# impromptuRong/hd_yolo

Hardware: NVIDIA B200
Metric: postproc_tiles_per_s (higher is better)
Workload: dtype f32

## Files before the change

### hd_yolo_b200/csrc/merge.cu

```cuda
#include "hdy_common.cuh"

namespace hdy {

enum : uint8_t { MS_UNKNOWN = 0, MS_KEPT = 1, MS_SUPPRESSED = 2, MS_DROPPED = 3, MS_REMOTE_UNKNOWN = 4 };

constexpr int kMergeThreads = 256;
constexpr int kMaxRounds = 64;
constexpr float kMergeCellMargin = 1.01f;
constexpr float kMergeMaxScaled = 1.0e6f;

constexpr int kExtBins = 128;
struct MergeStats {
  float ext_sum;
  unsigned ext_cnt;
  float cell_size;
  unsigned ext_hist[kExtBins];
  int unknown[kMaxRounds + 1];
  int rounds_run;
};

constexpr int kScanThreads = 1024;
constexpr int kScanItems = 4;
constexpr int kScanTile = kScanThreads * kScanItems;

// ... 546 lines not shown
    kept_dom = __any_sync(0xffffffffu, kept_dom);
    unk_dom = __any_sync(0xffffffffu, unk_dom);
    if (lane == 0) {
      if (kept_dom)
        vstate[p] = (uint8_t)MS_SUPPRESSED;
      else if (!unk_dom)
        vstate[p] = (uint8_t)MS_KEPT;
      else
        atomicAdd(&stats->unknown[round], 1);
    }
  }
}

__global__ void __launch_bounds__(kMergeThreads) merge_large_push_kernel(const float4* __restrict__ cbox,
                                                                         const uint64_t* __restrict__ ckey,
                                                                         uint8_t* cstate, const int* __restrict__ cell,
                                                                         const MergeStats* stats, int G, float thr,
                                                                         int round, uint32_t* __restrict__ blocked) {
  if (round > 0 && stats->unknown[round - 1] == 0) return;
  const int NB = G * G + 1;
  const int n_active = cell[NB - 1];
  const int large_begin = cell[NB - 2];
  const CellGeom g = cell_geom(stats);
  volatile uint8_t* vstate = cstate;
  const int lane = threadIdx.x & 31;
  const int warp = (blockIdx.x * blockDim.x + threadIdx.x) >> 5, n_warps = (gridDim.x * blockDim.x) >> 5;
  const uint32_t stamp = (uint32_t)round + 1u;
  for (int q = large_begin + warp; q < n_active; q += n_warps) {
    const uint8_t sq = vstate[q];
    if (sq != MS_KEPT && sq != MS_UNKNOWN && sq != MS_REMOTE_UNKNOWN) continue;
    const float4 bq = cbox[q];
    const uint64_t kq = ckey[q];
    auto visit = [&](int p) {
      if (kq < ckey[p] && vstate[p] == MS_UNKNOWN && iou_gt(bq, cbox[p], thr)) {
        if (sq == MS_KEPT)
          vstate[p] = (uint8_t)MS_SUPPRESSED;
        else
          blocked[p] = stamp;
      }
    };
    const float half = 0.5f * g.cell_size;
    const float fx0 = floorf((bq.x - half) * g.inv_cell), fx1 = floorf((bq.z + half) * g.inv_cell);
    const float fy0 = floorf((bq.y - half) * g.inv_cell), fy1 = floorf((bq.w + half) * g.inv_cell);
    const bool finite = fabsf(fx0) < 1.0e9f && fabsf(fx1) < 1.0e9f && fabsf(fy0) < 1.0e9f && fabsf(fy1) < 1.0e9f &&
                        fx1 >= fx0 && fy1 >= fy0;
    if (!finite) {
      for (int p = lane; p < large_begin; p += 32) visit(p);
    } else {
      const int ix0 = (int)fx0, iy0 = (int)fy0;
      const int nx = (int)fminf(fx1 - fx0 + 1.0f, (float)G), ny = (int)fminf(fy1 - fy0 + 1.0f, (float)G);
      const long long cells = (long long)nx * ny;
      for (long long c = lane; c < cells; c += 32) {
        const int cy = (int)(c / nx), cx = (int)(c - (long long)cy * nx);
        const int b = ((ix0 + cx) & (G - 1)) + ((iy0 + cy) & (G - 1)) * G;
        const int beg = b ? cell[b - 1] : 0, end = cell[b];
        for (int p = beg; p < end; ++p) visit(p);
      }
    }
  }
}

__global__ void merge_finish_kernel(const uint32_t* __restrict__ pos, const uint8_t* __restrict__ cstate,
                                    const long long* __restrict__ n_dev, long long n_max,
                                    uint8_t* __restrict__ state, int32_t* __restrict__ status) {
  const long long n = n_dev ? min(*n_dev, n_max) : n_max;
  bool bad = false;
  for (long long i = (long long)blockIdx.x * blockDim.x + threadIdx.x; i < n; i += (long long)gridDim.x * blockDim.x) {
    const uint32_t p = pos[i];
    if (p == 0xffffffffu) continue;
    uint8_t s = cstate[p];
    if (s == MS_UNKNOWN || s == MS_REMOTE_UNKNOWN) {
      s = MS_UNKNOWN;
      bad = true;
    }
    state[i] = s;
  }
  if (bad && status) atomicOr(status, HDY_STATUS_ROUNDS);
}

constexpr int kSelThreads = 256;
constexpr int kSelMaxBlocks = 4096;

__global__ void __launch_bounds__(kSelThreads) select_count_kernel(const uint8_t* __restrict__ state,
                                                                   const long long* __restrict__ n_dev,
                                                                   long long n_max, long long chunk,
                                                                   int* __restrict__ block_counts) {
  const long long n = n_dev ? min(*n_dev, n_max) : n_max;
  const long long lo = (long long)blockIdx.x * chunk, hi = min(lo + chunk, n);
  int c = 0;
  for (long long i = lo + threadIdx.x; i < hi; i += kSelThreads) c += state[i] == MS_KEPT;
  __shared__ int part[kSelThreads / 32];
#pragma unroll
  for (int o = 16; o > 0; o >>= 1) c += __shfl_xor_sync(0xffffffffu, c, o);
  if ((threadIdx.x & 31) == 0) part[threadIdx.x >> 5] = c;
  __syncthreads();
  if (threadIdx.x == 0) {
    int t = 0;
    for (int w = 0; w < kSelThreads / 32; ++w) t += part[w];
    block_counts[blockIdx.x] = t;
  }
}

__global__ void __launch_bounds__(1024) select_scan_kernel(int* __restrict__ block_counts, int nblocks,
                                                           int* __restrict__ count_out) {
  __shared__ int warp_tmp[33];
  int v[4], s = 0;
#pragma unroll
  for (int j = 0; j < 4; ++j) {
    const int i = threadIdx.x * 4 + j;
    v[j] = i < nblocks ? block_counts[i] : 0;
    s += v[j];
  }
  int total;
  int excl = block_scan_1024(s, warp_tmp, total);
#pragma unroll
  for (int j = 0; j < 4; ++j) {
    const int i = threadIdx.x * 4 + j;
    if (i < nblocks) block_counts[i] = excl;
    excl += v[j];
  }
  if (threadIdx.x == 0) *count_out = total;
}

__global__ void __launch_bounds__(kSelThreads) select_write_kernel(const uint8_t* __restrict__ state,
                                                                   const float* __restrict__ scores,
                                                                   const long long* __restrict__ n_dev,
                                                                   long long n_max, long long chunk,
                                                                   const int* __restrict__ block_offsets,
                                                                   uint64_t* __restrict__ keys) {
  __shared__ int wcount[kSelThreads / 32];
  const long long n = n_dev ? min(*n_dev, n_max) : n_max;
  const long long lo = (long long)blockIdx.x * chunk, hi = min(lo + chunk, n);
  const int lane = threadIdx.x & 31, warp = threadIdx.x >> 5;
  long long running = block_offsets[blockIdx.x];
  for (long long i0 = lo; i0 < hi; i0 += kSelThreads) {
    const long long i = i0 + threadIdx.x;
    const bool k = i < hi && state[i] == MS_KEPT;
    const unsigned m = __ballot_sync(0xffffffffu, k);
    if (lane == 0) wcount[warp] = __popc(m);
    __syncthreads();
    int before = 0, total = 0;
#pragma unroll
    for (int w = 0; w < kSelThreads / 32; ++w) {
      const int c = wcount[w];
      if (w < warp) before += c;
      total += c;
    }
    if (k) keys[running + before + __popc(m & ((1u << lane) - 1u))] = make_key(scores[i], (uint32_t)i);
    running += total;
    __syncthreads();
  }
}

constexpr int kSortThreads = 256;
constexpr int kSortPerWarp = 1024;
constexpr int kSortWarps = kSortThreads / 32;

__global__ void __launch_bounds__(kSortThreads) sort_hist_kernel(const uint64_t* __restrict__ keys,
                                                                  const int* __restrict__ n_dev, int n_max, int shift,
                                                                  int n_sub, int* __restrict__ hist) {
  __shared__ int h[kSortWarps][256];
  const int n = n_dev ? min(*n_dev, n_max) : n_max;
  const int warp = threadIdx.x >> 5, lane = threadIdx.x & 31;
  const int sub = blockIdx.x * kSortWarps + warp;
  for (int d = lane; d < 256; d += 32) h[warp][d] = 0;
  __syncwarp();
  const long long b = (long long)sub * kSortPerWarp;
  for (int k = lane; k < kSortPerWarp; k += 32)
    if (b + k < n) atomicAdd(&h[warp][(int)((keys[b + k] >> shift) & 255)], 1);
  __syncwarp();
  if (sub < n_sub)
    for (int d = lane; d < 256; d += 32) hist[(size_t)d * n_sub + sub] = h[warp][d];
}

__global__ void __launch_bounds__(kSortThreads) sort_scatter_kernel(const uint64_t* __restrict__ keys,
                                                                     const int* __restrict__ n_dev, int n_max,
                                                                     int shift, int n_sub, const int* __restrict__ hist,
                                                                     uint64_t* __restrict__ out) {
  __shared__ int base[kSortWarps][256];
  const int n = n_dev ? min(*n_dev, n_max) : n_max;
  const int warp = threadIdx.x >> 5, lane = threadIdx.x & 31;
  const int sub = blockIdx.x * kSortWarps + warp;
  if (sub >= n_sub) return;
  for (int d = lane; d < 256; d += 32) base[warp][d] = hist[(size_t)d * n_sub + sub];
  __syncwarp();
  const long long b = (long long)sub * kSortPerWarp;
  for (int k0 = 0; k0 < kSortPerWarp; k0 += 32) {
    const long long i = b + k0 + lane;
    const bool valid = i < n;
    const uint64_t key = valid ? keys[i] : 0;
    const int d = valid ? (int)((key >> shift) & 255) : 256 + lane;
    const unsigned peers = __match_any_sync(0xffffffffu, d);
    const int rank = __popc(peers & ((1u << lane) - 1u));
    int dst = 0;
    if (valid) dst = base[warp][d] + rank;
    __syncwarp();
    if (valid && rank == 0) base[warp][d] += __popc(peers);
    __syncwarp();
    if (valid) out[dst] = key;
  }
}

__global__ void merge_gather_kernel(const uint64_t* __restrict__ keys, const int* __restrict__ count, int max_det,
                                    const float4* __restrict__ boxes, const float* __restrict__ scores,
                                    const int64_t* __restrict__ labels, int64_t* __restrict__ out_idx,
                                    float4* __restrict__ out_boxes, float* __restrict__ out_scores,
                                    int64_t* __restrict__ out_labels, int* __restrict__ out_count) {
  const int k = min(*count, max_det);
  if (blockIdx.x == 0 && threadIdx.x == 0) *out_count = k;
  for (int j = blockIdx.x * blockDim.x + threadIdx.x; j < k; j += gridDim.x * blockDim.x) {
    const uint32_t i = key_index(keys[j]);
    if (out_idx) out_idx[j] = (int64_t)i;
    if (out_boxes) out_boxes[j] = boxes[i];
    if (out_scores) out_scores[j] = scores[i];
    if (out_labels && labels) out_labels[j] = labels[i];
  }
}

static inline unsigned blocks_for(long long n, int threads, int max_blocks = 148 * 16) {
  long long b = (n + threads - 1) / threads;
  if (b < 1) b = 1;
  if (b > max_blocks) b = max_blocks;
  return (unsigned)b;
}

constexpr int kSeamHdr = HDY_SEAM_HDR_WORDS, kSeamFar = HDY_SEAM_FAR_WORDS, kSeamRow = HDY_SEAM_ROW_WORDS;
constexpr int kSeamMaxWorld = HDY_SEAM_MAX_WORLD;
enum { SM_NTOTAL = 0, SM_MARGIN = 2, SM_GBASE = 3, SM_FLAGS = 4, SM_FAR_TOTAL = 5, SM_UNDECIDED = 8, SM_REP_OFF = 16,
       SM_OWN_SEAM = 88 };

__device__ __forceinline__ void atomic_min_float(float* addr, float v) {
  if (v >= 0.f)
    atomicMin(reinterpret_cast<int*>(addr), __float_as_int(v));
  else
    atomicMax(reinterpret_cast<unsigned*>(addr), __float_as_uint(v));
}
__device__ __forceinline__ void atomic_max_float(float* addr, float v) {
  if (v >= 0.f)
    atomicMax(reinterpret_cast<int*>(addr), __float_as_int(v));
  else
    atomicMin(reinterpret_cast<unsigned*>(addr), __float_as_uint(v));
}

__global__ void seam_summary_pack_kernel(long long n_local, const float* __restrict__ margin,
                                         const float4* __restrict__ far_boxes, const int32_t* __restrict__ far_tile,
                                         const int32_t* __restrict__ far_count, int far_list_capacity, int tile_base,
                                         int far_cap, int32_t* __restrict__ block) {
  const int k = blockIdx.x * blockDim.x + threadIdx.x;
  const int nf = far_count ? *far_count : 0;
  if (k == 0) {
    float* f = reinterpret_cast<float*>(block);
    const float big = 3.0e38f;
    f[0] = big, f[1] = big, f[2] = -big, f[3] = -big;
    f[4] = margin ? *margin : 0.f;
    block[5] = nf > far_list_capacity ? far_cap + 1 : nf;
    *reinterpret_cast<long long*>(block + 6) = n_local;
    for (int i = 8; i < kSeamHdr; ++i) block[i] = 0;
  }
  if (k < far_cap) {
    int32_t* e = block + kSeamHdr + k * kSeamFar;
    if (k < min(nf, far_list_capacity)) {
      const float4 b = far_boxes[k];
      e[0] = __float_as_int(b.x), e[1] = __float_as_int(b.y), e[2] = __float_as_int(b.z), e[3] = __float_as_int(b.w);
      e[4] = far_tile[k] + tile_base;
    } else {
      e[0] = e[1] = e[2] = e[3] = 0, e[4] = -1;
    }
    e[5] = e[6] = e[7] = 0;
  }
}

__global__ void seam_rect_kernel(const float4* __restrict__ boxes, long long n, float* __restrict__ rect) {
  const float big = 3.0e38f;
  float x1 = big, y1 = big, x2 = -big, y2 = -big;
  for (long long i = (long long)blockIdx.x * blockDim.x + threadIdx.x; i < n; i += (long long)gridDim.x * blockDim.x) {
    const float4 b = boxes[i];
    x1 = fminf(x1, fmaxf(b.x, -big)), y1 = fminf(y1, fmaxf(b.y, -big));
    x2 = fmaxf(x2, fminf(b.z, big)), y2 = fmaxf(y2, fminf(b.w, big));
  }
#pragma unroll
  for (int o = 16; o > 0; o >>= 1) {
    x1 = fminf(x1, __shfl_xor_sync(0xffffffffu, x1, o)), y1 = fminf(y1, __shfl_xor_sync(0xffffffffu, y1, o));
    x2 = fmaxf(x2, __shfl_xor_sync(0xffffffffu, x2, o)), y2 = fmaxf(y2, __shfl_xor_sync(0xffffffffu, y2, o));
  }
  if ((threadIdx.x & 31) == 0 && x2 >= x1) {
    atomic_min_float(rect + 0, x1), atomic_min_float(rect + 1, y1);
    atomic_max_float(rect + 2, x2), atomic_max_float(rect + 3, y2);
  }
}

struct SeamRects {
  float4 r[kSeamMaxWorld];
  int live[kSeamMaxWorld];
};
__device__ __forceinline__ void seam_load_rects(SeamRects& S, const int32_t* summaries, int world, int rank, int hb) {
  for (int q = threadIdx.x; q < world; q += blockDim.x) {
    const int32_t* h = summaries + (size_t)q * hb;
    S.r[q] = make_float4(__int_as_float(h[0]), __int_as_float(h[1]), __int_as_float(h[2]), __int_as_float(h[3]));
    S.live[q] = (q != rank) && (*reinterpret_cast<const long long*>(h + 6) > 0);
  }
  __syncthreads();
}
__device__ __forceinline__ bool seam_row(const float4& b, const SeamRects& S, int world) {
  bool s = false;
  for (int q = 0; q < world; ++q)
    s |= S.live[q] && (b.z >= S.r[q].x) && (b.x <= S.r[q].z) && (b.w >= S.r[q].y) && (b.y <= S.r[q].w);
  return s;
}

__global__ void __launch_bounds__(kSelThreads) seam_count_kernel(const float4* __restrict__ boxes, long long n,
                                                                 long long chunk, const int32_t* __restrict__ summaries,
                                                                 int world, int rank, int hb,
                                                                 int* __restrict__ block_counts) {
  __shared__ SeamRects S;
  __shared__ int part[kSelThreads / 32];
  seam_load_rects(S, summaries, world, rank, hb);
  const long long lo = (long long)blockIdx.x * chunk, hi = min(lo + chunk, n);
  int c = 0;
  for (long long i = lo + threadIdx.x; i < hi; i += kSelThreads) c += seam_row(boxes[i], S, world);
#pragma unroll
  for (int o = 16; o > 0; o >>= 1) c += __shfl_xor_sync(0xffffffffu, c, o);
  if ((threadIdx.x & 31) == 0) part[threadIdx.x >> 5] = c;
  __syncthreads();
  if (threadIdx.x == 0) {
    int t = 0;
    for (int w = 0; w < kSelThreads / 32; ++w) t += part[w];
    block_counts[blockIdx.x] = t;
  }
}

__global__ void __launch_bounds__(kSelThreads) seam_write_kernel(const float4* __restrict__ boxes,
                                                                 const float* __restrict__ scores, long long n,
                                                                 long long chunk, const int32_t* __restrict__ summaries,
                                                                 int world, int rank, int hb,
                                                                 const int* __restrict__ block_offsets, int seam_cap,
                                                                 int32_t* __restrict__ sel, int32_t* __restrict__ block) {
  __shared__ SeamRects S;
  __shared__ int wcount[kSelThreads / 32];
  seam_load_rects(S, summaries, world, rank, hb);
  long long gbase = 0;
  for (int q = 0; q < rank; ++q) gbase += *reinterpret_cast<const long long*>(summaries + (size_t)q * hb + 6);
  const long long lo = (long long)blockIdx.x * chunk, hi = min(lo + chunk, n);
  const int lane = threadIdx.x & 31, warp = threadIdx.x >> 5;
  long long running = block_offsets[blockIdx.x];
  for (long long i0 = lo; i0 < hi; i0 += kSelThreads) {
    const long long i = i0 + threadIdx.x;
    float4 b = make_float4(0.f, 0.f, 0.f, 0.f);
    bool k = false;
    if (i < hi) {
      b = boxes[i];
      k = seam_row(b, S, world);
    }
    const unsigned m = __ballot_sync(0xffffffffu, k);
    if (lane == 0) wcount[warp] = __popc(m);
    __syncthreads();
    int before = 0, total = 0;
#pragma unroll
    for (int w = 0; w < kSelThreads / 32; ++w) {
      const int c = wcount[w];
      if (w < warp) before += c;
      total += c;
    }
    const long long slot = running + before + __popc(m & ((1u << lane) - 1u));
    if (k && slot < seam_cap) {
      sel[slot] = (int32_t)i;
      int32_t* e = block + kSeamHdr + slot * kSeamRow;
      e[0] = __float_as_int(b.x), e[1] = __float_as_int(b.y), e[2] = __float_as_int(b.z), e[3] = __float_as_int(b.w);
      e[4] = __float_as_int(scores[i]);
// ... 268 lines not shown
      set_error("hdy_seam_select: %s", cudaGetErrorString(e));
      return HDY_ERR_CUDA;
    }
    return HDY_OK;
  }
  HDY_REQUIRE(boxes && scores && ((uintptr_t)boxes & 15) == 0, "hdy_seam_select: NULL or misaligned pointer");
  long long chunk = (n_local + kSelMaxBlocks - 1) / kSelMaxBlocks;
  chunk = ((chunk + kSelThreads - 1) / kSelThreads) * kSelThreads;
  if (chunk < 4 * kSelThreads) chunk = 4 * kSelThreads;
  const int nblocks = (int)((n_local + chunk - 1) / chunk);
  const float4* b4 = reinterpret_cast<const float4*>(boxes);
  const int hb = seam_hb(far_cap);
  seam_count_kernel<<<nblocks, kSelThreads, 0, st>>>(b4, n_local, chunk, summaries, world, rank, hb, block_scratch);
  select_scan_kernel<<<1, 1024, 0, st>>>(block_scratch, nblocks, block_scratch + kSelMaxBlocks);
  seam_block_header_kernel<<<1, 32, 0, st>>>(block_scratch + kSelMaxBlocks, block);
  seam_write_kernel<<<nblocks, kSelThreads, 0, st>>>(b4, scores, n_local, chunk, summaries, world, rank, hb,
                                                     block_scratch, seam_cap, sel, block);
  return check_launch("hdy_seam_select");
}

int hdy_seam_scatter(const int32_t* payloads, const int32_t* summaries, int world, int rank, int far_cap, int seam_cap,
                     int64_t n_local, int64_t rep_cap, float* boxes, float* scores, uint32_t* rep_gidx, int32_t* meta,
                     hdy_stream_t stream) {
  HDY_REQUIRE(world >= 1 && world <= kSeamMaxWorld && rank >= 0 && rank < world && far_cap >= 0 && seam_cap >= 0 &&
                  n_local >= 0 && rep_cap >= 0,
              "hdy_seam_scatter: bad arguments");
  HDY_REQUIRE(payloads && summaries && boxes && scores && rep_gidx && meta && ((uintptr_t)boxes & 15) == 0,
              "hdy_seam_scatter: NULL or misaligned pointer");
  dim3 grid((unsigned)(seam_cap / 1024 + 1), (unsigned)world);
  if (grid.x > 64) grid.x = 64;
  seam_scatter_kernel<<<grid, 256, 0, (cudaStream_t)stream>>>(payloads, summaries, world, rank, seam_hb(far_cap),
                                                            seam_pb(seam_cap), far_cap, seam_cap, n_local, rep_cap,
                                                            reinterpret_cast<float4*>(boxes), scores, rep_gidx, meta);
  return check_launch("hdy_seam_scatter");
}

int hdy_seam_dirty_tiles(const int32_t* summaries, int world, int far_cap, const float* tile_rois, int n_tiles,
                         uint8_t* dirty, hdy_stream_t stream) {
  HDY_REQUIRE(world >= 1 && far_cap >= 0 && n_tiles >= 0, "hdy_seam_dirty_tiles: bad sizes");
  if (n_tiles == 0) return HDY_OK;
  HDY_REQUIRE(summaries && tile_rois && dirty && ((uintptr_t)tile_rois & 15) == 0,
              "hdy_seam_dirty_tiles: NULL or misaligned pointer");
  seam_dirty_tiles_kernel<<<(unsigned)((n_tiles + 127) / 128), 128, 0, (cudaStream_t)stream>>>(
      summaries, world, seam_hb(far_cap), far_cap, reinterpret_cast<const float4*>(tile_rois), n_tiles, dirty);
  return check_launch("hdy_seam_dirty_tiles");
}

int hdy_seam_build(const float* boxes, const float* scores, const uint32_t* rep_gidx, const int32_t* meta,
                   const int32_t* tile_id, int tile_base, const float* tile_cores, const uint8_t* tile_dirty,
                   int64_t n_max, int64_t n_local, float conf_thres, float iou_thres, uint8_t* state, void* workspace,
                   size_t workspace_bytes, hdy_stream_t stream) {
  HDY_REQUIRE(meta && rep_gidx, "hdy_seam_build: NULL pointer");
  MergeIn in;
  in.boxes = reinterpret_cast<const float4*>(boxes);
  in.scores = scores;
  in.rep_gidx = rep_gidx;
  in.gidx_base_dev = reinterpret_cast<const uint32_t*>(meta + SM_GBASE);
  in.tile_base = tile_base;
  in.tile_id = tile_id;
  in.tile_cores = reinterpret_cast<const float4*>(tile_cores);
  in.tile_dirty = tile_dirty;
  in.margin = reinterpret_cast<const float*>(meta + SM_MARGIN);
  in.n_dev = reinterpret_cast<const long long*>(meta + SM_NTOTAL);
  in.n_max = n_max;
  in.n_local = n_local;
  in.conf = conf_thres;
  in.thr = iou_thres;
  return merge_build_common("hdy_seam_build", in, tile_cores, state, workspace, workspace_bytes, (cudaStream_t)stream);
}

int hdy_seam_export(void* workspace, int64_t n_max, const uint8_t* state, const int32_t* sel, const int32_t* my_block,
                    int seam_cap, uint8_t* out, hdy_stream_t stream) {
  HDY_REQUIRE(workspace && n_max >= 0 && seam_cap >= 0, "hdy_seam_export: bad arguments");
  if (seam_cap == 0 || n_max == 0) return HDY_OK;
  HDY_REQUIRE(state && sel && my_block && out, "hdy_seam_export: NULL pointer");
  MergeWs w = merge_layout(workspace, n_max);
  seam_export_kernel<<<blocks_for(seam_cap, 256, 148), 256, 0, (cudaStream_t)stream>>>(w.pos, w.cstate, state, sel,
                                                                                    my_block, seam_cap, out);
  return check_launch("hdy_seam_export");
}

int hdy_seam_import(void* workspace, int64_t n_max, int64_t n_local, const uint8_t* states, const int32_t* payloads,
                    int32_t* meta, int world, int rank, int seam_cap, int exchange, hdy_stream_t stream) {
  HDY_REQUIRE(workspace && n_max >= 0 && n_local >= 0 && world >= 1 && world <= kSeamMaxWorld && rank >= 0 &&
                  rank < world && seam_cap >= 0 && exchange >= 0,
              "hdy_seam_import: bad arguments");
  HDY_REQUIRE(states && payloads && meta, "hdy_seam_import: NULL pointer");
  MergeWs w = merge_layout(workspace, n_max > 0 ? n_max : 1);
  dim3 grid((unsigned)(seam_cap / 1024 + 1), (unsigned)world);
  if (grid.x > 64) grid.x = 64;
  seam_import_kernel<<<grid, 256, 0, (cudaStream_t)stream>>>(w.pos, w.cstate, n_local, states, payloads,
                                                           seam_pb(seam_cap), meta, world, rank, seam_cap, exchange);
  return check_launch("hdy_seam_import");
}

int hdy_merge_rounds(void* workspace, int64_t n_max, float iou_thres, int first_round, int n_rounds,
                     hdy_stream_t stream) {
  HDY_REQUIRE(workspace && n_max >= 0, "hdy_merge_rounds: bad arguments");
  HDY_REQUIRE(first_round >= 0 && n_rounds >= 0 && first_round + n_rounds <= kMaxRounds,
              "hdy_merge_rounds: at most %d rounds in total", kMaxRounds);
  if (n_max == 0) return HDY_OK;
  MergeWs w = merge_layout(workspace, n_max);
  const unsigned blocks = blocks_for(n_max, kMergeThreads, 148 * 8);
  for (int r = first_round; r < first_round + n_rounds; ++r) {
    merge_large_push_kernel<<<148 * 2, kMergeThreads, 0, (cudaStream_t)stream>>>(w.cbox, w.ckey, w.cstate, w.cell,
                                                                                 w.stats, w.G, iou_thres, r, w.blocked);
    merge_round_kernel<<<blocks, kMergeThreads, 0, (cudaStream_t)stream>>>(w.cbox, w.ckey, w.cstate, w.cell, w.stats,
                                                                           w.G, iou_thres, r, w.blocked, w.ctile);
    merge_round_large_kernel<<<148 * 2, kMergeThreads, 0, (cudaStream_t)stream>>>(w.cbox, w.ckey, w.cstate, w.cell,
                                                                                  w.stats, w.G, iou_thres, r);
  }
  return check_launch("hdy_merge_rounds");
}

int hdy_merge_finish(void* workspace, const int64_t* n_dev, int64_t n_max, uint8_t* state, int32_t* status,
                     hdy_stream_t stream) {
  HDY_REQUIRE(workspace && n_max >= 0, "hdy_merge_finish: bad arguments");
  if (n_max == 0) return HDY_OK;
  HDY_REQUIRE(state != nullptr, "hdy_merge_finish: state is NULL");
  MergeWs w = merge_layout(workspace, n_max);
  merge_finish_kernel<<<blocks_for(n_max, 256), 256, 0, (cudaStream_t)stream>>>(
      w.pos, w.cstate, reinterpret_cast<const long long*>(n_dev), n_max, state, status);
  return check_launch("hdy_merge_finish");
}

int hdy_merge_nms(const float* boxes, const float* scores, const int32_t* tile_id, const float* tile_cores,
                  const uint8_t* tile_dirty, const float* margin, const int64_t* n_dev, int64_t n_max, float conf_thres,
                  float iou_thres,
                  int max_rounds, uint8_t* state, int32_t* status, void* workspace, size_t workspace_bytes,
                  hdy_stream_t stream) {
  HDY_REQUIRE(max_rounds >= 1 && max_rounds <= kMaxRounds, "hdy_merge_nms: max_rounds out of range [1,%d]", kMaxRounds);
  MergeIn in;
  in.boxes = reinterpret_cast<const float4*>(boxes);
  in.scores = scores;
  in.rep_gidx = nullptr;
  in.gidx_base_dev = nullptr;
  in.tile_base = 0;
  in.tile_id = tile_id;
  in.tile_cores = reinterpret_cast<const float4*>(tile_cores);
  in.tile_dirty = tile_dirty;
  in.margin = margin;
  in.n_dev = reinterpret_cast<const long long*>(n_dev);
  in.n_max = n_max;
  in.n_local = n_max;
  in.conf = conf_thres;
  in.thr = iou_thres;
  int rc = merge_build_common("hdy_merge_nms", in, tile_cores, state, workspace, workspace_bytes, (cudaStream_t)stream);
  if (rc) return rc;
  rc = hdy_merge_rounds(workspace, n_max, iou_thres, 0, max_rounds, stream);
  if (rc) return rc;
  return hdy_merge_finish(workspace, n_dev, n_max, state, status, stream);
}

size_t hdy_sort_workspace_bytes(int64_t n_max) {
  if (n_max <= 0) return 256;
  const long long n_sub = (n_max + kSortPerWarp - 1) / kSortPerWarp;
  const long long hist = 256 * n_sub;
  return align256((size_t)hist * 4) + align256(scan_scratch_ints(hist) * 4);
}

int hdy_sort_keys_bytes(uint64_t* keys, uint64_t* tmp, const int32_t* n_dev, int64_t n_max, int first_byte,
                        int n_bytes, void* workspace, size_t workspace_bytes, hdy_stream_t stream) {
  HDY_REQUIRE(first_byte >= 0 && n_bytes >= 0 && first_byte + n_bytes <= 8 && (n_bytes & 1) == 0,
              "hdy_sort_keys_bytes: bytes [%d, %d) -- an even number of bytes inside the key", first_byte,
              first_byte + n_bytes);
  HDY_REQUIRE(n_max >= 0 && n_max < (1ll << 31), "hdy_sort_keys_bytes: bad size");
  if (n_max == 0) return HDY_OK;
  HDY_REQUIRE(keys && tmp && workspace && workspace_bytes >= hdy_sort_workspace_bytes(n_max),
              "hdy_sort_keys_bytes: NULL pointer or workspace too small");
  cudaStream_t st = (cudaStream_t)stream;
  const int n_sub = (int)((n_max + kSortPerWarp - 1) / kSortPerWarp);
  const long long hist_n = 256ll * n_sub;
  int* hist = static_cast<int*>(workspace);
  int* scratch = reinterpret_cast<int*>(static_cast<unsigned char*>(workspace) + align256((size_t)hist_n * 4));
  const unsigned blocks = (unsigned)((n_sub + kSortWarps - 1) / kSortWarps);
  uint64_t* src = keys;
  uint64_t* dst = tmp;
  for (int pass = first_byte; pass < first_byte + n_bytes; ++pass) {
    sort_hist_kernel<<<blocks, kSortThreads, 0, st>>>(src, n_dev, (int)n_max, pass * 8, n_sub, hist);
    int rc = device_exclusive_scan(hist, hist_n, scratch, nullptr, st);
    if (rc) return rc;
    sort_scatter_kernel<<<blocks, kSortThreads, 0, st>>>(src, n_dev, (int)n_max, pass * 8, n_sub, hist, dst);
    uint64_t* t = src;
    src = dst;
    dst = t;
  }
  return check_launch("hdy_sort_keys_bytes");
}

int hdy_merge_select_ordered(const uint8_t* state, const float* scores, const int64_t* n_dev, int64_t n_max,
                             uint64_t* keys, int32_t* count, int32_t* block_scratch, hdy_stream_t stream) {
  HDY_REQUIRE(n_max >= 0 && n_max < (1ll << 31) && count && block_scratch, "hdy_merge_select_ordered: bad arguments");
  cudaStream_t st = (cudaStream_t)stream;
  if (n_max == 0) {
    cudaError_t e = cudaMemsetAsync(count, 0, 4, st);
    if (e != cudaSuccess) {
      set_error("hdy_merge_select_ordered: %s", cudaGetErrorString(e));
      return HDY_ERR_CUDA;
    }
    return HDY_OK;
  }
  HDY_REQUIRE(state && scores && keys, "hdy_merge_select_ordered: NULL pointer");
  long long chunk = (n_max + kSelMaxBlocks - 1) / kSelMaxBlocks;
  chunk = ((chunk + kSelThreads - 1) / kSelThreads) * kSelThreads;
  if (chunk < 4 * kSelThreads) chunk = 4 * kSelThreads;
  const int nblocks = (int)((n_max + chunk - 1) / chunk);
  const long long* nd = reinterpret_cast<const long long*>(n_dev);
  select_count_kernel<<<nblocks, kSelThreads, 0, st>>>(state, nd, n_max, chunk, block_scratch);
  select_scan_kernel<<<1, 1024, 0, st>>>(block_scratch, nblocks, count);
  select_write_kernel<<<nblocks, kSelThreads, 0, st>>>(state, scores, nd, n_max, chunk, block_scratch, keys);
  return check_launch("hdy_merge_select_ordered");
}

int hdy_merge_gather(const uint64_t* keys, const int32_t* count, int64_t max_det, const float* boxes,
                     const float* scores, const int64_t* labels, int64_t* out_idx, float* out_boxes,
                     float* out_scores, int64_t* out_labels, int32_t* out_count, hdy_stream_t stream) {
  HDY_REQUIRE(max_det >= 0 && max_det < (1ll << 31) && keys && count && out_count, "hdy_merge_gather: bad arguments");
  HDY_REQUIRE((!out_boxes || boxes) && (!out_scores || scores), "hdy_merge_gather: output without its source");
  HDY_REQUIRE((((uintptr_t)boxes | (uintptr_t)out_boxes) & 15) == 0, "hdy_merge_gather: box arrays must be 16-byte aligned");
  merge_gather_kernel<<<blocks_for(max_det > 0 ? max_det : 1, 256), 256, 0, (cudaStream_t)stream>>>(
      keys, count, (int)max_det, reinterpret_cast<const float4*>(boxes), scores, labels, out_idx,
      reinterpret_cast<float4*>(out_boxes), out_scores, out_labels, out_count);
  return check_launch("hdy_merge_gather");
}

}
```

### hd_yolo_b200/slide.py

```python
from __future__ import annotations

import ctypes as C
from typing import Dict, List, Optional, Sequence, Tuple

import torch

from . import _lib
from ._lib import HdyError, ptr
from .ops import DetectBatch, _Scratch, _aligned16, _call, _conf_thr_f32, _iou_thr_f32, _need_cuda, _stream

__all__ = ["sliding_window_scanner", "tile_cores", "merge_outputs", "rescale_outputs", "scale_coords", "clip_coords",
           "merge_nms", "ensemble_merge", "Ensemble", "SlideAccumulator", "sort_keys", "kept_digest", "fold_digest",
           "mask_digest",
           "STATE_KEPT", "STATE_SUPPRESSED", "STATE_DROPPED"]

STATE_UNKNOWN, STATE_KEPT, STATE_SUPPRESSED, STATE_DROPPED = 0, 1, 2, 3
AFFINE_UNPAD, AFFINE_SCALE, AFFINE_CLIP, AFFINE_ROUND = 1, 2, 4, 8
_ws = _Scratch()


def _pair(v):
    return (v, v) if isinstance(v, (int, float)) else (v[0], v[1])


def sliding_window_scanner(image_size, roi_size=None, overlap=0) -> torch.Tensor:
    if roi_size is None:
        return torch.tensor([[0., 0., image_size[0], image_size[1]]], dtype=torch.float32)
    h, w = _pair(image_size)
    roi_h, roi_w = _pair(roi_size)
    xs = torch.arange(0, w, roi_w - overlap, dtype=torch.float32) if w > roi_w else torch.zeros(1)
    ys = torch.arange(0, h, roi_h - overlap, dtype=torch.float32) if h > roi_h else torch.zeros(1)
    x0 = xs.repeat(len(ys))
    y0 = ys.repeat_interleave(len(xs))
    out = torch.stack((x0, y0, x0 + roi_w, y0 + roi_h), 1)
    out[:, 0::2] = out[:, 0::2].clamp(min=0, max=w)
    out[:, 1::2] = out[:, 1::2].clamp(min=0, max=h)
    return out


def tile_cores(rois: torch.Tensor) -> torch.Tensor:
    r = rois.detach().cpu().to(torch.float64)
    big = 3.0e38
    out = torch.empty((len(r), 4), dtype=torch.float64)
    for lo, hi in ((0, 2), (1, 3)):
        starts = torch.unique(r[:, lo])
        ends = torch.stack([r[r[:, lo] == s, hi].max() for s in starts])
        idx = torch.searchsorted(starts, r[:, lo].contiguous())
        prev_end = torch.cat([torch.tensor([-big], dtype=torch.float64), ends[:-1]])
        prev_end = torch.cummax(prev_end, 0).values
        next_start = torch.cat([starts[1:], torch.tensor([big], dtype=torch.float64)])
        out[:, lo] = prev_end[idx]
        out[:, hi] = next_start[idx]
    return out.to(torch.float32)


def _affine(rows: torch.Tensor, pad_x, pad_y, gain, scale, clip_w, clip_h, flags):
    _need_cuda(rows, "coords")
    if rows.dim() != 2 or rows.shape[1] < 4 or rows.stride(1) != 1:
        raise HdyError("coords must be [n, >=4] with unit stride along columns")
    if rows.shape[0]:
        _call("hdy_affine_boxes", ptr(rows), rows.shape[0], rows.stride(0), float(pad_x), float(pad_y), float(gain),
              float(scale), float(clip_w), float(clip_h), flags, _stream())
    return rows


def clip_coords(boxes: torch.Tensor, shape) -> None:
    _affine(boxes, 0, 0, 1, 1, shape[1], shape[0], AFFINE_CLIP)


def scale_coords(img1_shape, coords: torch.Tensor, img0_shape, ratio_pad=None, round_: bool = False) -> torch.Tensor:
    img1_shape, img0_shape = _pair(img1_shape), _pair(img0_shape)
    if ratio_pad is None:
        gain = min(img1_shape[0] / img0_shape[0], img1_shape[1] / img0_shape[1])
        pad = (img1_shape[1] - img0_shape[1] * gain) / 2, (img1_shape[0] - img0_shape[0] * gain) / 2
    else:
        gain = ratio_pad[0][0]
        pad = ratio_pad[1]
    return _affine(coords, pad[0], pad[1], gain, 1, img0_shape[1], img0_shape[0],
                   AFFINE_UNPAD | AFFINE_CLIP | (AFFINE_ROUND if round_ else 0))


def rescale_outputs(r: Dict[str, torch.Tensor], scale: float = 1.0) -> Dict[str, torch.Tensor]:
    if scale != 1.0:
        _affine(r['boxes'], 0, 0, 1, scale, 0, 0, AFFINE_SCALE)
    return r


def merge_nms(boxes: torch.Tensor, scores: torch.Tensor, conf_thres: float, iou_thres: float,
              tile_id: Optional[torch.Tensor] = None, cores: Optional[torch.Tensor] = None,
              margin: Optional[torch.Tensor] = None, n_dev: Optional[torch.Tensor] = None,
              max_rounds: int = 8, dirty: Optional[torch.Tensor] = None) -> torch.Tensor:
    _need_cuda(boxes, "boxes")
    _need_cuda(scores, "scores")
    n = boxes.shape[0]
    if boxes.dim() != 2 or boxes.shape[1] != 4 or scores.shape != (n,):
        raise HdyError("boxes must be [n,4] and scores [n]")
    dev = boxes.device
    state = torch.empty((n,), dtype=torch.uint8, device=dev)
    if n == 0:
        return state
    boxes = _aligned16(boxes.contiguous())
    scores = scores.contiguous()
    lib = _lib.load()
    wbytes = lib.hdy_merge_workspace_bytes(n)
    ws = _ws.get(dev, "merge", wbytes)
    status = torch.zeros((1,), dtype=torch.int32, device=dev)
    use_cores = cores is not None
    if use_cores and (tile_id is None or margin is None):
        raise HdyError("the interior shortcut needs tile_id, cores and margin")
    rounds = max_rounds
    while True:
        _call("hdy_merge_nms", ptr(boxes), ptr(scores), ptr(tile_id) if use_cores else None,
              ptr(cores) if use_cores else None, ptr(dirty) if use_cores else None,
              ptr(margin) if use_cores else None, ptr(n_dev), n,
              _conf_thr_f32(conf_thres), _iou_thr_f32(iou_thres), rounds, ptr(state), ptr(status), ptr(ws), wbytes,
              _stream(), launches=8 + 3 * rounds)
        if not int(status.item()) & _lib.HDY_STATUS_ROUNDS:
            return state
        if rounds >= 64:
            raise HdyError("merge NMS did not converge in 64 rounds")
        rounds, _ = min(64, rounds * 2), status.zero_()


def dirty_tiles(far_boxes: torch.Tensor, far_tile: torch.Tensor, far_count: torch.Tensor,
                rois: torch.Tensor) -> torch.Tensor:
    n_tiles = int(rois.shape[0])
    dirty = torch.empty((max(n_tiles, 1),), dtype=torch.uint8, device=rois.device)
    _call("hdy_merge_dirty_tiles", ptr(far_boxes), ptr(far_tile), ptr(far_count), int(far_boxes.shape[0]),
          ptr(_aligned16(rois.contiguous())), n_tiles, ptr(dirty), _stream())
    return dirty


def sort_keys(keys: torch.Tensor, n_dev: Optional[torch.Tensor] = None, first_byte: int = 0,
              n_bytes: int = 8) -> torch.Tensor:
    if not keys.is_cuda or keys.dtype != torch.int64 or not keys.is_contiguous():
        raise HdyError("keys must be a contiguous CUDA int64 tensor")
    n = keys.numel()
    if n:
        lib = _lib.load()
        wbytes = lib.hdy_sort_workspace_bytes(n)
        ws = _ws.get(keys.device, "sort", wbytes)
        tmp = _ws.get(keys.device, "sort_tmp", n * 8)
        _call("hdy_sort_keys_bytes", ptr(keys), ptr(tmp), ptr(n_dev), n, int(first_byte), int(n_bytes), ptr(ws), wbytes,
              _stream(), launches=int(n_bytes) * 5)
    return keys


def _order_keys(state, scores, n: int, count: torch.Tensor) -> torch.Tensor:
    dev = scores.device
    keys = torch.empty((max(n, 1),), dtype=torch.int64, device=dev)
    if n == 0:
        count.zero_()
        return keys
    blk = _ws.get(dev, "select_blocks", 4096 * 4)
    _call("hdy_merge_select_ordered", ptr(state), ptr(scores), None, n, ptr(keys), ptr(count), ptr(blk), _stream(),
          launches=3)
    sort_keys(keys, n_dev=count, first_byte=4, n_bytes=4)
    return keys


def _gather_ordered(keys, count, k_all: int, max_det: int, boxes, scores, labels):
    dev = boxes.device
    k = min(int(k_all), int(max_det))
    idx = torch.empty((k,), dtype=torch.int64, device=dev)
    ob = torch.empty((k, 4), dtype=torch.float32, device=dev)
    os_ = torch.empty((k,), dtype=torch.float32, device=dev)
    ol = torch.empty((k,), dtype=torch.int64, device=dev) if labels is not None else None
    oc = torch.empty((1,), dtype=torch.int32, device=dev)
    if k:
        _call("hdy_merge_gather", ptr(keys), ptr(count), k, ptr(boxes), ptr(scores), ptr(labels), ptr(idx), ptr(ob),
              ptr(os_), ptr(ol), ptr(oc), _stream())
    return idx, ob, os_, ol


def _kept_in_order(state, boxes, scores, labels, max_det: int, n_dev=None):
    n = boxes.shape[0]
    count = torch.empty((1,), dtype=torch.int32, device=boxes.device)
    keys = _order_keys(state, scores, n, count)
    return _gather_ordered(keys, count, int(count.item()), max_det, boxes, scores, labels)


def kept_digest(state: torch.Tensor, base: int = 0) -> torch.Tensor:
    idx = torch.nonzero(state == STATE_KEPT).flatten().to(torch.int64) + int(base)
    h = idx * -7046029254386353131
    h = h ^ (h >> 31)
    h = h * -4658895280553007687
    h = h ^ (h >> 29)
    lo = (h & 0xffffffff).sum()
    hi = ((h >> 32) & 0xffffffff).sum()
    return torch.stack([torch.tensor(idx.numel(), dtype=torch.int64, device=state.device), lo, hi])


def fold_digest(t: torch.Tensor) -> Dict[str, object]:
    c, lo, hi = [int(v) for v in t.tolist()]
    return {"kept": c, "hash": f"{(lo + (hi << 32)) & 0xffffffffffffffff:016x}"}


def mask_digest(masks, state: torch.Tensor, base: int = 0, chunk_rows: int = 1 << 19) -> torch.Tensor:
    dev = state.device
    all_rows = torch.nonzero(state == STATE_KEPT).flatten()
    acc = torch.zeros((3,), dtype=torch.int64, device=dev)
    for c0 in range(0, int(all_rows.numel()), chunk_rows):
        rows = all_rows[c0:c0 + chunk_rows]
        g = masks.geom[rows].to(torch.int64)
        words = ((g[:, 2] + 31) >> 5) * g[:, 3]
        total = int(words.sum())
        if total == 0:
            continue
        owner = torch.repeat_interleave(torch.arange(rows.numel(), device=dev), words)
        start = torch.cumsum(words, 0) - words
        j = torch.arange(total, device=dev) - start[owner]
        w = masks.bits[masks.offsets[rows][owner] + j].to(torch.int64) & 0xffffffff
        h = ((rows[owner] + int(base)) * 1000003 + j) * -7046029254386353131
        h = (h ^ (h >> 31)) + w * -4658895280553007687
        h = h ^ (h >> 29)
        pop = w - ((w >> 1) & 0x55555555)
        pop = (pop & 0x33333333) + ((pop >> 2) & 0x33333333)
        pop = ((((pop + (pop >> 4)) & 0x0f0f0f0f) * 0x01010101) >> 24) & 0xff
        acc += torch.stack([pop.sum(), (h & 0xffffffff).sum(), ((h >> 32) & 0xffffffff).sum()])
    return acc


def merge_outputs(r: List[Dict[str, torch.Tensor]]) -> Dict[str, torch.Tensor]:
    if not len(r):
        raise HdyError("merge_outputs needs at least one tile")
    dev = r[0]['boxes'].device
    _need_cuda(r[0]['boxes'], "boxes")
    counts_h = [int(t['boxes'].shape[0]) for t in r]
    bs, md = len(r), max(max(counts_h), 1)
    n = sum(counts_h)
    res = {'labels': torch.cat([t['labels'] for t in r]), 'scores': torch.cat([t['scores'] for t in r])}
    cat = _aligned16(torch.cat([t['boxes'] for t in r]).contiguous())
    rois = torch.stack([torch.as_tensor(t['roi'], dtype=torch.float32).reshape(-1)[:4].cpu() for t in r]).to(dev)
    out = torch.empty((n, 4), dtype=torch.float32, device=dev)
    if n:
        counts = torch.tensor(counts_h, dtype=torch.int32).to(dev)
        offs = torch.tensor([0] + counts_h[:-1], dtype=torch.int64).cumsum(0).to(dev)
        tile_of = torch.repeat_interleave(torch.arange(bs, device=dev), counts.long())
        slot = torch.arange(n, device=dev) - offs[tile_of]
        padded = torch.zeros((bs, md, 4), dtype=torch.float32, device=dev)
        padded[tile_of, slot] = cat
        cursor = torch.zeros((1,), dtype=torch.int64, device=dev)
        tile_offsets = torch.empty((bs + 1,), dtype=torch.int64, device=dev)
        status = torch.zeros((1,), dtype=torch.int32, device=dev)
        for b0 in range(0, bs, 65535):
            b1 = min(bs, b0 + 65535)
            _call("hdy_merge_append", ptr(padded[b0:b1]), None, None, None, ptr(counts[b0:b1]), ptr(rois[b0:b1]), b1 - b0, md,
                  b0, 1.0, n, ptr(out), None, None, None, ptr(cursor), ptr(tile_offsets[b0:]), ptr(status), _stream(),
                  launches=2)
    res = {'boxes': out, **res}
    if 'masks' in r[0]:
        res['masks'] = torch.cat([t['masks'] for t in r])
    return res


def ensemble_merge(x: List[Dict[str, Dict[str, torch.Tensor]]], nms_params: Dict[str, float]):
    task_ids = set().union(*x)
    res: Dict[str, Dict[str, torch.Tensor]] = {}
    conf, iou, max_det = nms_params['conf_thres'], nms_params['iou_thres'], int(nms_params['max_det'])
    for task_id in task_ids:
        parts = [r[task_id] for r in x if task_id in r]
        boxes = torch.cat([p['boxes'] for p in parts])
        scores = torch.cat([p['scores'] for p in parts])
        labels = torch.cat([p['labels'] for p in parts])
        masks = None
        if any('masks' in p for p in parts):
            ref = [p['masks'] for p in parts if 'masks' in p][0]
            masks = torch.cat([p['masks'] if 'masks' in p else torch.zeros(ref.shape[1:]).to(ref.device, ref.dtype)
                               for p in parts])
        if scores.dim() != 1:
            raise HdyError("Ensemble.merge handles single-label outputs (scores [n]); the reference's multi-label "
                           "merge is unfinished (yolo.py:145)")
        lab64 = labels.to(torch.int64).contiguous()
        boxes = _aligned16(boxes.contiguous().float())
        state = merge_nms(boxes, scores.contiguous(), conf, iou)
        idx, ob, os_, ol = _kept_in_order(state, boxes, scores.contiguous(), lab64, max_det)
        out = {'boxes': ob, 'scores': os_, 'labels': ol.to(labels.dtype)}
        if masks is not None:
            out['masks'] = masks[idx]
        res[task_id] = out
    return res


class Ensemble:

    def __init__(self, models=(), nms_params: Dict[str, float] = {}):
        self.models = list(models)
        self.nms_params = self.get_nms_params(nms_params)

    def get_nms_params(self, args={}):
        default_args = {'conf_thres': 0.15, 'iou_thres': 0.45, 'max_det': 300}
        return {k: float(args.get(k, v)) for k, v in default_args.items()}

    def merge(self, x):
        return ensemble_merge(x, self.nms_params)


# ... 148 lines not shown
```

Before: 161,400.

## Replace per-pass radix sort with onesweep decoupled-lookback sort and batch gather

Replaces the per-byte histogram, device scan and scatter passes with a single upfront multi-byte histogram, a small bases kernel, and one onesweep kernel per byte. That kernel uses decoupled lookback over per-tile status words and stages keys in shared memory so global writes are coalesced. This removes the repeated scans and kernel launches for each digit pass. The gather kernel now processes several rows per thread and reads the score from the sort key instead of the scores array. The lookback spin relies on forward progress between tiles, acquired in ticket order, and the gather assumes key scores are nonzero and finite.

```diff
diff --git a/hd_yolo_b200/csrc/merge.cu b/hd_yolo_b200/csrc/merge.cu
--- a/hd_yolo_b200/csrc/merge.cu
+++ b/hd_yolo_b200/csrc/merge.cu
@@ -722,68 +722,230 @@
   }
 }
 
+constexpr int kHistThreads = 256;
+constexpr int kHistItems = 4;
+constexpr int kHistCopies = 4;
 constexpr int kSortThreads = 256;
-constexpr int kSortPerWarp = 1024;
 constexpr int kSortWarps = kSortThreads / 32;
-
-__global__ void __launch_bounds__(kSortThreads) sort_hist_kernel(const uint64_t* __restrict__ keys,
-                                                                  const int* __restrict__ n_dev, int n_max, int shift,
-                                                                  int n_sub, int* __restrict__ hist) {
-  __shared__ int h[kSortWarps][256];
+constexpr int kSortItems = 12;
+constexpr int kSortWarpKeys = kSortItems * 32;
+constexpr int kSortTile = kSortThreads * kSortItems;
+constexpr int kSortMaxBytes = 8;
+constexpr size_t kSortHdrBytes = (kSortMaxBytes * 256 + kSortMaxBytes) * 4;
+
+__device__ __forceinline__ void status_store(unsigned long long* p, unsigned long long v) {
+  asm volatile("st.relaxed.gpu.global.u64 [%0], %1;" ::"l"(p), "l"(v) : "memory");
+}
+__device__ __forceinline__ unsigned long long status_load(const unsigned long long* p) {
+  unsigned long long v;
+  asm volatile("ld.relaxed.gpu.global.u64 %0, [%1];" : "=l"(v) : "l"(p) : "memory");
+  return v;
+}
+
+__global__ void __launch_bounds__(kHistThreads) sort_hist_kernel(const uint64_t* __restrict__ keys,
+                                                                  const int* __restrict__ n_dev, int n_max,
+                                                                  int first_byte, int n_bytes,
+                                                                  unsigned* __restrict__ counts) {
+  extern __shared__ unsigned hcnt[];
   const int n = n_dev ? min(*n_dev, n_max) : n_max;
-  const int warp = threadIdx.x >> 5, lane = threadIdx.x & 31;
-  const int sub = blockIdx.x * kSortWarps + warp;
-  for (int d = lane; d < 256; d += 32) h[warp][d] = 0;
-  __syncwarp();
-  const long long b = (long long)sub * kSortPerWarp;
-  for (int k = lane; k < kSortPerWarp; k += 32)
-    if (b + k < n) atomicAdd(&h[warp][(int)((keys[b + k] >> shift) & 255)], 1);
-  __syncwarp();
-  if (sub < n_sub)
-    for (int d = lane; d < 256; d += 32) hist[(size_t)d * n_sub + sub] = h[warp][d];
-}
-
-__global__ void __launch_bounds__(kSortThreads) sort_scatter_kernel(const uint64_t* __restrict__ keys,
-                                                                     const int* __restrict__ n_dev, int n_max,
-                                                                     int shift, int n_sub, const int* __restrict__ hist,
-                                                                     uint64_t* __restrict__ out) {
-  __shared__ int base[kSortWarps][256];
+  for (int i = threadIdx.x; i < n_bytes * 256 * kHistCopies; i += kHistThreads) hcnt[i] = 0u;
+  __syncthreads();
+  const int copy = threadIdx.x % kHistCopies;
+  const long long step = (long long)gridDim.x * kHistThreads * kHistItems;
+  for (long long i0 = (long long)blockIdx.x * kHistThreads * kHistItems + threadIdx.x; i0 < n; i0 += step) {
+    uint64_t k[kHistItems];
+#pragma unroll
+    for (int e = 0; e < kHistItems; ++e) {
+      const long long i = i0 + (long long)e * kHistThreads;
+      k[e] = i < n ? keys[i] >> (8 * first_byte) : 0ull;
+    }
+#pragma unroll
+    for (int e = 0; e < kHistItems; ++e) {
+      if (i0 + (long long)e * kHistThreads >= n) break;
+      for (int b = 0; b < n_bytes; ++b)
+        atomicAdd(&hcnt[(b * 256 + (int)((k[e] >> (8 * b)) & 255ull)) * kHistCopies + copy], 1u);
+    }
+  }
+  __syncthreads();
+  for (int i = threadIdx.x; i < n_bytes * 256; i += kHistThreads) {
+    unsigned s = 0u;
+#pragma unroll
+    for (int c = 0; c < kHistCopies; ++c) s += hcnt[i * kHistCopies + c];
+    if (s) atomicAdd(&counts[i], s);
+  }
+}
+
+__global__ void __launch_bounds__(kSortMaxBytes * 32) sort_bases_kernel(unsigned* __restrict__ counts, int n_bytes) {
+  const int w = threadIdx.x >> 5, lane = threadIdx.x & 31;
+  if (w >= n_bytes) return;
+  unsigned* c = counts + w * 256 + lane * 8;
+  unsigned v[8], sum = 0u;
+#pragma unroll
+  for (int j = 0; j < 8; ++j) {
+    v[j] = c[j];
+    sum += v[j];
+  }
+  unsigned incl = sum;
+#pragma unroll
+  for (int o = 1; o < 32; o <<= 1) {
+    const unsigned u = __shfl_up_sync(0xffffffffu, incl, o);
+    if (lane >= o) incl += u;
+  }
+  unsigned run = incl - sum;
+#pragma unroll
+  for (int j = 0; j < 8; ++j) {
+    c[j] = run;
+    run += v[j];
+  }
+}
+
+__global__ void __launch_bounds__(kSortThreads, 3) sort_onesweep_kernel(const uint64_t* __restrict__ src,
+                                                                         uint64_t* __restrict__ dst,
+                                                                         const int* __restrict__ n_dev, int n_max,
+                                                                         int shift, unsigned stamp,
+                                                                         const unsigned* __restrict__ bases,
+                                                                         unsigned* __restrict__ ticket,
+                                                                         unsigned long long* __restrict__ status) {
+  __shared__ uint64_t stage[kSortTile];
+  __shared__ uint16_t whist[kSortWarps][256];
+  __shared__ int dstart[256];
+  __shared__ int gshift[256];
+  __shared__ int wsum[kSortWarps];
+  __shared__ int s_tile;
+  const int t = threadIdx.x, lane = t & 31, w = t >> 5;
+  if (t == 0) s_tile = (int)atomicAdd(ticket, 1u);
+  {
+    uint32_t* z = reinterpret_cast<uint32_t*>(&whist[0][0]);
+    for (int i = t; i < kSortWarps * 128; i += kSortThreads) z[i] = 0u;
+  }
+  __syncthreads();
+  const int tile = s_tile;
   const int n = n_dev ? min(*n_dev, n_max) : n_max;
-  const int warp = threadIdx.x >> 5, lane = threadIdx.x & 31;
-  const int sub = blockIdx.x * kSortWarps + warp;
-  if (sub >= n_sub) return;
-  for (int d = lane; d < 256; d += 32) base[warp][d] = hist[(size_t)d * n_sub + sub];
-  __syncwarp();
-  const long long b = (long long)sub * kSortPerWarp;
-  for (int k0 = 0; k0 < kSortPerWarp; k0 += 32) {
-    const long long i = b + k0 + lane;
-    const bool valid = i < n;
-    const uint64_t key = valid ? keys[i] : 0;
-    const int d = valid ? (int)((key >> shift) & 255) : 256 + lane;
-    const unsigned peers = __match_any_sync(0xffffffffu, d);
-    const int rank = __popc(peers & ((1u << lane) - 1u));
-    int dst = 0;
-    if (valid) dst = base[warp][d] + rank;
+  const long long lo = (long long)tile * kSortTile;
+  if (lo >= n) return;
+  const int in_tile = (int)min((long long)kSortTile, (long long)n - lo);
+
+  uint64_t k[kSortItems];
+  unsigned loc[kSortItems / 2];
+#pragma unroll
+  for (int e = 0; e < kSortItems; ++e) {
+    const int i = w * kSortWarpKeys + e * 32 + lane;
+    k[e] = i < in_tile ? src[lo + i] : 0ull;
+  }
+  uint16_t* wh = whist[w];
+#pragma unroll
+  for (int e = 0; e < kSortItems; ++e) {
+    const bool valid = w * kSortWarpKeys + e * 32 + lane < in_tile;
+    const int d = (int)((k[e] >> shift) & 255ull);
+    unsigned peers = __ballot_sync(0xffffffffu, valid);
+#pragma unroll
+    for (int bit = 0; bit < 8; ++bit) {
+      const unsigned m = __ballot_sync(0xffffffffu, (d >> bit) & 1);
+      peers &= ((d >> bit) & 1) ? m : ~m;
+    }
+    const int r = __popc(peers & ((1u << lane) - 1u));
+    const int pre = wh[d];
     __syncwarp();
-    if (valid && rank == 0) base[warp][d] += __popc(peers);
+    if (valid && r == 0) wh[d] = (uint16_t)(pre + __popc(peers));
     __syncwarp();
-    if (valid) out[dst] = key;
-  }
-}
-
-__global__ void merge_gather_kernel(const uint64_t* __restrict__ keys, const int* __restrict__ count, int max_det,
-                                    const float4* __restrict__ boxes, const float* __restrict__ scores,
-                                    const int64_t* __restrict__ labels, int64_t* __restrict__ out_idx,
-                                    float4* __restrict__ out_boxes, float* __restrict__ out_scores,
-                                    int64_t* __restrict__ out_labels, int* __restrict__ out_count) {
+    loc[e / 2] = (e & 1) ? loc[e / 2] | (unsigned)(pre + r) << 16 : (unsigned)(pre + r);
+  }
+  __syncthreads();
+
+  const int d = t;
+  int cnt = 0;
+#pragma unroll
+  for (int j = 0; j < kSortWarps; ++j) {
+    const int c = whist[j][d];
+    whist[j][d] = (uint16_t)cnt;
+    cnt += c;
+  }
+  unsigned long long* my = status + (size_t)tile * 256 + d;
+  status_store(my, ((unsigned long long)(tile == 0 ? stamp + 1 : stamp) << 32) | (unsigned)cnt);
+
+  int incl = cnt;
+#pragma unroll
+  for (int o = 1; o < 32; o <<= 1) {
+    const int u = __shfl_up_sync(0xffffffffu, incl, o);
+    if (lane >= o) incl += u;
+  }
+  if (lane == 31) wsum[w] = incl;
+  __syncthreads();
+  int start = incl - cnt;
+  for (int j = 0; j < w; ++j) start += wsum[j];
+  dstart[d] = start;
+  __syncthreads();
+
+#pragma unroll
+  for (int e = 0; e < kSortItems; ++e) {
+    if (w * kSortWarpKeys + e * 32 + lane < in_tile) {
+      const int dd = (int)((k[e] >> shift) & 255ull);
+      stage[dstart[dd] + whist[w][dd] + (int)((loc[e / 2] >> (16 * (e & 1))) & 0xffffu)] = k[e];
+    }
+  }
+
+  unsigned excl = 0u;
+  if (tile > 0) {
+    for (int j = tile - 1;; --j) {
+      unsigned long long s;
+      do {
+        s = status_load(status + (size_t)j * 256 + d);
+      } while ((unsigned)(s >> 32) < stamp);
+      excl += (unsigned)s;
+      if ((unsigned)(s >> 32) != stamp) break;
+    }
+    status_store(my, ((unsigned long long)(stamp + 1) << 32) | (excl + (unsigned)cnt));
+  }
+  gshift[d] = (int)(bases[d] + excl) - start;
+  __syncthreads();
+
+#pragma unroll 4
+  for (int p = t; p < in_tile; p += kSortThreads) {
+    const uint64_t key = stage[p];
+    dst[gshift[(int)((key >> shift) & 255ull)] + p] = key;
+  }
+}
+
+constexpr int kGatherThreads = 256;
+constexpr int kGatherRows = 4;
+
+__global__ void __launch_bounds__(kGatherThreads, 4) merge_gather_kernel(
+    const uint64_t* __restrict__ keys, const int* __restrict__ count, int max_det, const float4* __restrict__ boxes,
+    const float* __restrict__ scores, const int64_t* __restrict__ labels, int64_t* __restrict__ out_idx,
+    float4* __restrict__ out_boxes, float* __restrict__ out_scores, int64_t* __restrict__ out_labels,
+    int* __restrict__ out_count) {
   const int k = min(*count, max_det);
   if (blockIdx.x == 0 && threadIdx.x == 0) *out_count = k;
-  for (int j = blockIdx.x * blockDim.x + threadIdx.x; j < k; j += gridDim.x * blockDim.x) {
-    const uint32_t i = key_index(keys[j]);
-    if (out_idx) out_idx[j] = (int64_t)i;
-    if (out_boxes) out_boxes[j] = boxes[i];
-    if (out_scores) out_scores[j] = scores[i];
-    if (out_labels && labels) out_labels[j] = labels[i];
+  const bool want_labels = out_labels && labels;
+  const long long step = (long long)gridDim.x * kGatherThreads * kGatherRows;
+  for (long long j0 = (long long)blockIdx.x * kGatherThreads * kGatherRows + threadIdx.x; j0 < k; j0 += step) {
+    uint64_t key[kGatherRows];
+#pragma unroll
+    for (int r = 0; r < kGatherRows; ++r) {
+      const long long j = j0 + r * kGatherThreads;
+      key[r] = j < k ? keys[j] : 0ull;
+    }
+    float4 box[kGatherRows];
+    int64_t lab[kGatherRows];
+    float sc[kGatherRows];
+#pragma unroll
+    for (int r = 0; r < kGatherRows; ++r) {
+      if (j0 + r * kGatherThreads >= k) break;
+      const uint32_t i = key_index(key[r]);
+      if (out_boxes) box[r] = boxes[i];
+      if (want_labels) lab[r] = labels[i];
+      sc[r] = key_score(key[r]);
+      if (out_scores && !(sc[r] != 0.f && sc[r] == sc[r])) sc[r] = scores[i];
+    }
+#pragma unroll
+    for (int r = 0; r < kGatherRows; ++r) {
+      const long long j = j0 + r * kGatherThreads;
+      if (j >= k) break;
+      if (out_idx) out_idx[j] = (int64_t)key_index(key[r]);
+      if (out_boxes) out_boxes[j] = box[r];
+      if (out_scores) out_scores[j] = sc[r];
+      if (want_labels) out_labels[j] = lab[r];
+    }
   }
 }
 
@@ -1358,11 +1520,11 @@
   return hdy_merge_finish(workspace, n_dev, n_max, state, status, stream);
 }
 
+static inline long long sort_tiles(long long n_max) { return (n_max + kSortTile - 1) / kSortTile; }
+
 size_t hdy_sort_workspace_bytes(int64_t n_max) {
   if (n_max <= 0) return 256;
-  const long long n_sub = (n_max + kSortPerWarp - 1) / kSortPerWarp;
-  const long long hist = 256 * n_sub;
-  return align256((size_t)hist * 4) + align256(scan_scratch_ints(hist) * 4);
+  return align256(kSortHdrBytes) + align256((size_t)sort_tiles(n_max) * 256 * 8);
 }
 
 int hdy_sort_keys_bytes(uint64_t* keys, uint64_t* tmp, const int32_t* n_dev, int64_t n_max, int first_byte,
@@ -1374,19 +1536,26 @@
   if (n_max == 0) return HDY_OK;
   HDY_REQUIRE(keys && tmp && workspace && workspace_bytes >= hdy_sort_workspace_bytes(n_max),
               "hdy_sort_keys_bytes: NULL pointer or workspace too small");
+  if (n_bytes == 0) return HDY_OK;
   cudaStream_t st = (cudaStream_t)stream;
-  const int n_sub = (int)((n_max + kSortPerWarp - 1) / kSortPerWarp);
-  const long long hist_n = 256ll * n_sub;
-  int* hist = static_cast<int*>(workspace);
-  int* scratch = reinterpret_cast<int*>(static_cast<unsigned char*>(workspace) + align256((size_t)hist_n * 4));
-  const unsigned blocks = (unsigned)((n_sub + kSortWarps - 1) / kSortWarps);
+  const long long tiles = sort_tiles(n_max);
+  unsigned* counts = static_cast<unsigned*>(workspace);
+  unsigned* tickets = counts + kSortMaxBytes * 256;
+  auto* status = reinterpret_cast<unsigned long long*>(static_cast<unsigned char*>(workspace) + align256(kSortHdrBytes));
+  cudaError_t e = cudaMemsetAsync(workspace, 0, align256(kSortHdrBytes) + (size_t)tiles * 256 * 8, st);
+  if (e != cudaSuccess) {
+    set_error("hdy_sort_keys_bytes: %s", cudaGetErrorString(e));
+    return HDY_ERR_CUDA;
+  }
+  sort_hist_kernel<<<blocks_for(n_max, kHistThreads * kHistItems, 148 * 8), kHistThreads,
+                     (size_t)n_bytes * 256 * kHistCopies * 4, st>>>(keys, n_dev, (int)n_max, first_byte, n_bytes,
+                                                                     counts);
+  sort_bases_kernel<<<1, kSortMaxBytes * 32, 0, st>>>(counts, n_bytes);
   uint64_t* src = keys;
   uint64_t* dst = tmp;
-  for (int pass = first_byte; pass < first_byte + n_bytes; ++pass) {
-    sort_hist_kernel<<<blocks, kSortThreads, 0, st>>>(src, n_dev, (int)n_max, pass * 8, n_sub, hist);
-    int rc = device_exclusive_scan(hist, hist_n, scratch, nullptr, st);
-    if (rc) return rc;
-    sort_scatter_kernel<<<blocks, kSortThreads, 0, st>>>(src, n_dev, (int)n_max, pass * 8, n_sub, hist, dst);
+  for (int p = 0; p < n_bytes; ++p) {
+    sort_onesweep_kernel<<<(unsigned)tiles, kSortThreads, 0, st>>>(src, dst, n_dev, (int)n_max, (first_byte + p) * 8,
+                                                                   2u * p + 1u, counts + p * 256, tickets + p, status);
     uint64_t* t = src;
     src = dst;
     dst = t;
@@ -1424,7 +1593,8 @@
   HDY_REQUIRE(max_det >= 0 && max_det < (1ll << 31) && keys && count && out_count, "hdy_merge_gather: bad arguments");
   HDY_REQUIRE((!out_boxes || boxes) && (!out_scores || scores), "hdy_merge_gather: output without its source");
   HDY_REQUIRE((((uintptr_t)boxes | (uintptr_t)out_boxes) & 15) == 0, "hdy_merge_gather: box arrays must be 16-byte aligned");
-  merge_gather_kernel<<<blocks_for(max_det > 0 ? max_det : 1, 256), 256, 0, (cudaStream_t)stream>>>(
+  merge_gather_kernel<<<blocks_for(max_det, kGatherThreads * kGatherRows, 148 * 4), kGatherThreads, 0,
+                        (cudaStream_t)stream>>>(
       keys, count, (int)max_det, reinterpret_cast<const float4*>(boxes), scores, labels, out_idx,
       reinterpret_cast<float4*>(out_boxes), out_scores, out_labels, out_count);
   return check_launch("hdy_merge_gather");
diff --git a/hd_yolo_b200/slide.py b/hd_yolo_b200/slide.py
--- a/hd_yolo_b200/slide.py
+++ b/hd_yolo_b200/slide.py
@@ -142,7 +142,7 @@
         ws = _ws.get(keys.device, "sort", wbytes)
         tmp = _ws.get(keys.device, "sort_tmp", n * 8)
         _call("hdy_sort_keys_bytes", ptr(keys), ptr(tmp), ptr(n_dev), n, int(first_byte), int(n_bytes), ptr(ws), wbytes,
-              _stream(), launches=int(n_bytes) * 5)
+              _stream(), launches=int(n_bytes) + 3)
     return keys
 
 
```

Measured after the change: 164,100, median of 6. 1.7% higher.
